# nutdb/nutdb

Hardware: AMD Instinct MI355X
Metric: rows/sec filter->group-by on 1e9-row i64/f64; achieved HBM GB/s vs peak (higher is better)
Workload: dtype i64+f64; 1 GPU; tpch_q1_shape_filter_groupby; columns=6 x 8 B (i64/f64), groups=6, bytes_per_row=48, rows_per_gpu=1000000000, parallelism=single GPU, gpu=AMD Radeon Graphics, kernel_launches=387

## Files before the change

nutdb_amd/csrc/agg_kernel.hpp:

```cpp
#pragma once

#include "agg_ops.hpp"

namespace nut {

enum { CTL_CLAIMED = 0, CTL_SPECIAL = 1, CTL_LOCK = 2, CTL_NDENSE = 3 };
constexpr uint32_t kNoDense = 0xFFFFFFFFu;
constexpr uint32_t kDirect = 256;

struct LTable {
  uint64_t *slot, *agg;
  i64x2 *k12;
  uint32_t *did, *dslot, *ctl;
  uint32_t *dmap;
  uint64_t *priv;
  uint32_t *spill;
  uint32_t *shist;
};

__host__ __device__ inline size_t lds_layout(uint32_t cap, int nk, int na, bool privm, int P, int bd,
                                             size_t *o_k12, size_t *o_did, size_t *o_dslot, size_t *o_ctl,
                                             size_t *o_priv) {
  const size_t stride = cap + 1;
  size_t o = stride * 8 * (1 + (size_t)na);
// ... 434 lines not shown
          }
        }
      });
    }
  }
  if (p.sp_counts) {
    spill_rows<NK, S>(p, lt, kk1, kk2, sl, av, vm);
    return;
  }
#pragma unroll
  for (int r = 0; r < R; ++r) {
    if (sl[r] == -1 && NK == 1 && p.dense) {
      atomicOr(&p.gt->ctl[1], 4u);
    } else if (sl[r] == -1) {
      uint64_t g[8] = {0, 0, 0, 0, 0, 0, 0, 0};
      uint32_t m = 0;
#pragma unroll
      for (int a = 0; a < S::MA && a < 8; ++a) g[a] = av[a][r], m |= vm[a][r] ? 1u << a : 0u;
      g_row<NK>(p.gt, (int64_t)kk1[r], (int64_t)kk2[r], m, g[0], g[1], g[2], g[3], g[4], g[5], g[6], g[7]);
    }
  }
}

template <int NK, bool PRIV, int BD, class S, int VEC>
__global__ __launch_bounds__(BD) void agg_kernel(AggArgs p) {
  extern __shared__ __attribute__((aligned(16))) uint64_t smem[];
  const uint32_t cap = p.lds_cap;
  const uint32_t stride = cap + 1;
  const int na = S::na(p);
  LTable lt;
  {
    size_t o_k12, o_did, o_dslot, o_ctl, o_priv;
    lds_layout(cap, NK, na, PRIV, p.priv, BD, &o_k12, &o_did, &o_dslot, &o_ctl, &o_priv);
    char *b = (char *)smem;
    lt.slot = (uint64_t *)b;
    lt.agg = lt.slot + stride;
    lt.k12 = (i64x2 *)(b + o_k12);
    lt.did = PRIV ? (uint32_t *)(b + o_did) : nullptr;
    lt.dslot = (uint32_t *)(b + o_dslot);
    lt.dmap = PRIV ? lt.dslot + kPrivMax : nullptr;
    lt.ctl = (uint32_t *)(b + o_ctl);
    lt.priv = (uint64_t *)(b + o_priv);
  }
  __shared__ uint32_t s_spill;
  __shared__ uint32_t s_shist[256];
  lt.spill = &s_spill;
// ... 163 lines not shown
        continue;
      }
      if (base == ~0ull) continue;
      const uint64_t pos = base + r;
      t.slot[pos] = wd;
#pragma unroll
      for (int a = 0; a < S::MA; ++a)
        if (a < na) t.agg[a * gstr + pos] = lt.agg[a * stride + s];
    }
    return;
  }
  for (uint32_t s = threadIdx.x; s < stride; s += BD) {
    const uint64_t wd = lt.slot[s];
    const bool occ = s < cap ? wd != kEmpty : lt.ctl[CTL_SPECIAL] != 0u;
    if (!occ) continue;
    const int64_t k1 = NK == 1 ? (int64_t)(s < cap ? wd : kEmpty) : lt.k12[s].x;
    const int64_t k2 = NK == 1 ? 0 : lt.k12[s].y;
    const int64_t gs = g_find<NK>(t, key_hash<NK>(k1, k2), k1, k2);
    if (gs < 0) continue;
#pragma unroll
    for (int a = 0; a < S::MA; ++a)
      if (a < na) agg_merge_word(&t.agg[a * gstr + gs], S::kind(p, a), lt.agg[a * stride + s]);
  }
}

}
```

nutdb_amd/csrc/agg_ops.hpp:

```cpp
#pragma once

#include "gtable.hpp"

namespace nut {

constexpr int kPrivMax = 8;
constexpr int kMaxCols = NUT_MAX_PROG_COLS;
constexpr int kMaxConst = 64;

struct AggArgs {
  uint64_t n;
  const uint64_t *keys[2];
  const uint64_t *pred_col[NUT_MAX_PRED];
  uint64_t pred_k[NUT_MAX_PRED];
  int32_t pred_type[NUT_MAX_PRED];
  int32_t pred_op[NUT_MAX_PRED];
  const uint64_t *val_col[kMaxCols];
  int32_t npred, nvals, naggs;
  uint32_t kinds;
  int32_t expr[NUT_MAX_AGGS];
  int32_t arg[NUT_MAX_AGGS][3];
  uint32_t lds_cap;
  uint32_t lds_limit;
  int32_t lds_log2;
  int32_t priv;
  int32_t vec;
  int32_t nokey;
  int32_t pred_nset[NUT_MAX_PRED];
  uint64_t pred_set[NUT_MAX_PRED][NUT_MAX_SET];
  uint64_t kc[kMaxConst];
  const GTable *gt;
  uint64_t *sp_cols[3 + NUT_MAX_VALS];
  unsigned long long *sp_counts;
  unsigned long long *sp_hist;
  uint64_t sp_region;
  int32_t sp_map[NUT_MAX_AGGS];
  const uint64_t *seg_off;
  const uint64_t *seg_end;
  const uint64_t *seg_cut;
  int32_t dense, pad_;
  unsigned long long *dcount;
  uint64_t dregion, dbase;
};

struct NoProg {
  static constexpr bool kProg = false;
  template <class V>
  __device__ static bool where(const AggArgs &, const V &, int, bool &) { return true; }
  template <class V>
  __device__ static uint64_t value(const AggArgs &, int, const V &, int, bool &) { return 0; }
  template <class V>
  __device__ static bool valid(const AggArgs &, int, const V &, int, bool &) { return true; }
};

template <class S>
__host__ __device__ constexpr int col_type(int c) {
  if constexpr (S::kProg) return (int)((S::kColTypes >> (4 * c)) & 15u);
  else return NUT_T_I64;
}
template <class S>
__host__ __device__ constexpr bool shape_narrow() {
  for (int c = 0; c < S::MV; ++c)
    if (type_width(col_type<S>(c)) < 8) return true;
  return false;
}
// ... 184 lines not shown
```

nutdb_amd/csrc/aggregate.hip:

```cpp
#include <stdlib.h>
#include <string.h>

#include <algorithm>
#include <chrono>
#include <mutex>
#include <thread>
#include <vector>

#include "agg_kernel.hpp"
#include "gpart.hpp"
#include "fold.hpp"
#include "heavy.hpp"
#include "sort.hpp"
#include "jit.hpp"
#include "select_kernel.hpp"

using namespace nut;

struct nut_groups {
  nut_ctx *ctx = nullptr;
  int nk = 1, naggs = 0;
  int32_t kinds[NUT_MAX_AGGS] = {0};
  GTable gt{};
  GTable *dev_gt = nullptr;
  void *mem = nullptr;
  size_t mem_bytes = 0;
  unsigned long long *dev_cursors = nullptr;
  uint64_t *dev_segbase = nullptr;
  bool dense = false;
  uint32_t ctl_cache[4] = {0, 0, 0, 0};
  bool ctl_valid = false;
};

namespace {

int ilog2(uint64_t v) {
  int r = 0;
  while ((1ull << r) < v) ++r;
  return r;
}

uint32_t pack_kinds(const int32_t *k, int n) {
  uint32_t p = 0;
  for (int a = 0; a < n; ++a) p |= (uint32_t)(k[a] & 15) << (4 * a);
  return p;
}

nut_status validate(const nut_agg_spec *s) {
  if (!s) return fail(NUT_ERR_INVALID_ARG, "nut_groupby: spec is NULL");
  if (s->nkeys < 0 || s->nkeys > 2) return fail(NUT_ERR_UNSUPPORTED, "nut_groupby: 0, 1 or 2 key columns supported");
  if (s->npred < 0 || s->npred > NUT_MAX_PRED) return fail(NUT_ERR_UNSUPPORTED, "nut_groupby: too many predicate terms");
  if (s->nvals < 0 || s->nvals > NUT_MAX_VALS) return fail(NUT_ERR_UNSUPPORTED, "nut_groupby: too many value columns");
  if (s->naggs < 0 || s->naggs > NUT_MAX_AGGS) return fail(NUT_ERR_UNSUPPORTED, "nut_groupby: too many aggregates");
  for (int k = 0; k < NUT_MAX_KEYS; ++k) {
// ... 69 lines not shown
        return fail(NUT_ERR_UNSUPPORTED, "nut_groupby: arithmetic expressions need f64 columns");
    }
  }
  return NUT_OK;
}

int32_t kind_of(const nut_agg_spec *s, int a) {
  int op = s->agg_op[a];
  if (op == NUT_AGG_COUNT) return AK_COUNT;
  bool i64 = s->agg_expr[a] == NUT_EX_COL && s->val_type[s->agg_arg[a][0]] == NUT_T_I64;
  if (s->prog_mode) {
    int32_t t = NUT_PT_F64;
    (void)prog_check(&s->agg_val[a], s->prog_col_type, s->nprog_cols, &t);
    i64 = t != NUT_PT_F64;
  }
  switch (op) {
    case NUT_AGG_SUM: return i64 ? AK_SUM_I64 : AK_SUM_F64;
    case NUT_AGG_MIN: return i64 ? AK_MIN_I64 : AK_MIN_F64;
    default: return i64 ? AK_MAX_I64 : AK_MAX_F64;
  }
}

nut_status alloc_table(nut_groups *g, uint64_t cap) {
  g->ctl_valid = false;
  const uint64_t stride = cap + 1;
  const uint64_t arena = g->nk == 2 ? cap + 65536 : 0;
  size_t off = 0;
  auto carve = [&](size_t bytes) {
    size_t o = off;
    off += (bytes + 255) & ~size_t(255);
    return o;
  };
  size_t o_slot = carve(stride * 8);
  size_t o_agg = carve(stride * 8 * (size_t)std::max(g->naggs, 1));
  size_t o_a1 = carve(arena * 8 + 8);
  size_t o_a2 = carve(arena * 8 + 8);
  size_t o_ctl = carve(64);
  const int nsh_log2 = cap >= (1ull << 18) ? 8 : 0;
  const uint32_t nsh = 1u << nsh_log2;
  size_t o_sh = carve((size_t)nsh * 2 * 16 * 4);
  size_t o_gt = carve(sizeof(GTable));
  size_t o_cur = carve(64 * 8);
  size_t o_seg = carve(128 * 8);
  if (!(g->mem && g->mem_bytes >= off)) {
    if (g->mem) (void)hipFree(g->mem);
    g->mem = nullptr;
    nut_status ps = pool_take(g->ctx, off, &g->mem, &g->mem_bytes);
    if (ps) return ps;
  }
  char *b = (char *)g->mem;
  GTable &t = g->gt;
  t.slot = (uint64_t *)(b + o_slot);
  t.agg = (uint64_t *)(b + o_agg);
  t.ak1 = (int64_t *)(b + o_a1);
  t.ak2 = (int64_t *)(b + o_a2);
  t.ctl = (uint32_t *)(b + o_ctl);
  t.shard = (uint32_t *)(b + o_sh);
  t.nsh_log2 = nsh_log2;
  t.cap = cap;
  t.log2cap = ilog2(cap);
  t.limit = (uint32_t)std::min<uint64_t>(cap - cap / 4, 0xFFFFFFF0ull);
  t.arena_cap = (uint32_t)std::min<uint64_t>(arena, 0xFFFFFFF0ull);
  t.limit_sh = nsh == 1 ? t.limit : t.limit / nsh + t.limit / nsh / 16;
  t.arena_sh = t.arena_cap / nsh;
  t.naggs = g->naggs;
  t.kinds = pack_kinds(g->kinds, g->naggs);
  g->dev_gt = (GTable *)(b + o_gt);
  g->dev_cursors = (unsigned long long *)(b + o_cur);
  g->dev_segbase = (uint64_t *)(b + o_seg);
  hipStream_t st = g->ctx->stream;
  NUT_HIP(hipMemsetAsync(t.ctl, 0, 64, st));
  NUT_HIP(hipMemsetAsync(t.shard, 0, (size_t)nsh * 2 * 16 * 4, st));
  NUT_HIP(hipMemcpyAsync(g->dev_gt, &g->gt, sizeof(GTable), hipMemcpyHostToDevice, st));
  uint64_t blocks = std::min<uint64_t>((stride + 255) / 256, (uint64_t)g->ctx->num_cus * 8);
  hipLaunchKernelGGL(gtable_init_kernel, dim3((unsigned)blocks), dim3(256), 0, st, (const GTable *)g->dev_gt, g->nk);
  NUT_HIP(hipGetLastError());
  return NUT_OK;
}

nut_status read_ctl(nut_groups *g, uint32_t *ctl4) {
  if (g->ctl_valid) {
    memcpy(ctl4, g->ctl_cache, 16);
    return NUT_OK;
  }
  nut_ctx *c = g->ctx;
  hipLaunchKernelGGL(gtable_sum_kernel, dim3(1), dim3(256), 0, c->stream, (const GTable *)g->dev_gt);
  NUT_HIP(hipGetLastError());
  NUT_HIP(hipMemcpyAsync(c->host_pinned, g->gt.ctl, 16, hipMemcpyDeviceToHost, c->stream));
  NUT_HIP(hipStreamSynchronize(c->stream));
  memcpy(ctl4, c->host_pinned, 16);
  memcpy(g->ctl_cache, ctl4, 16);
  g->ctl_valid = true;
  return NUT_OK;
}

using KernelFn = void (*)(AggArgs);
enum { SHAPE_GENERIC = 0, SHAPE_Q1, SHAPE_SUM, SHAPE_SUMCOUNT, SHAPE_ALL4 };

template <class S>
bool shape_matches(const nut_agg_spec *s, const int32_t *kinds, const AggArgs &a) {
  if (s->npred != S::MP || s->nvals != S::MV || s->naggs != S::MA) return false;
  for (int i = 0; i < S::MA; ++i) {
    if (kinds[i] != (int)((S::kKinds >> (4 * i)) & 15u)) return false;
    if (a.expr[i] != (int)((S::kExprs >> (4 * i)) & 15u)) return false;
    const int nargs = a.expr[i] == NUT_EX_COL ? 1 : a.expr[i] == NUT_EX_MUL_1M_1P ? 3 : 2;
    for (int j = 0; j < 3; ++j) {
      int want = (int)((S::kArgs >> (6 * i + 2 * j)) & 3u);
// ... 63 lines not shown
constexpr int kPrivShapes[3][2] = {{192, 2}, {128, 3}, {128, 4}};
struct PrivShape {
  int shape = -1;
  double ms[3] = {-1, -1, -1};
  double cost_ms = 0;
};
static PrivShape g_priv_shape[64];
static std::mutex g_priv_mu;
static PrivShape priv_shape_of(int dev) {
  std::lock_guard<std::mutex> lk(g_priv_mu);
  return dev >= 0 && dev < 64 ? g_priv_shape[dev] : PrivShape{};
}

constexpr size_t kAggLdsMax = 160 * 1024 - 2048;
uint32_t agg_lcap(nut_ctx *c, int nk, int na, uint64_t group_hint, bool seg) {
  const uint64_t want = group_hint ? (uint64_t)c->opt[seg ? NUT_OPT_GB_SEG_SLOTS : NUT_OPT_AGG_SLOTS] * group_hint : 4096;
  uint32_t lcap = 32;
  while (lcap < want && lds_bytes(lcap * 2, nk, na, false, 0, kBdShared) <= kAggLdsMax) lcap *= 2;
  return group_hint > 8ull * lcap ? 0 : lcap;
}

nut_status launch_agg(nut_groups *g, const nut_agg_spec *s, uint64_t group_hint, const int32_t *kinds,
                      LaunchExtra *ex = nullptr) {
  g->ctl_valid = false;
  nut_ctx *c = g->ctx;
  if (s->n == 0) return NUT_OK;
  AggArgs a;
  memset(&a, 0, sizeof(a));
  a.n = s->n;
  a.nokey = s->nkeys == 0 ? 1 : 0;
  a.keys[0] = (const uint64_t *)(s->nkeys && !s->key_prog[0].n ? s->keys[0] : nullptr);
  a.keys[1] = s->nkeys == 2 && !s->key_prog[1].n ? (const uint64_t *)s->keys[1] : a.keys[0];
  a.npred = s->npred;
  for (int t = 0; t < s->npred; ++t) {
    a.pred_col[t] = (const uint64_t *)s->pred_col[t];
    a.pred_type[t] = s->pred_type[t];
    a.pred_op[t] = s->pred_op[t];
    if (s->pred_type[t] == NUT_T_I64) a.pred_k[t] = (uint64_t)s->pred_i64[t];
    else memcpy(&a.pred_k[t], &s->pred_f64[t], 8);
    if (s->pred_op[t] >= NUT_IN) {
      a.pred_nset[t] = s->pred_nset[t];
      for (int i = 0; i < s->pred_nset[t]; ++i) a.pred_set[t][i] = (uint64_t)s->pred_set[t][i];
    }
  }
  a.nvals = s->nvals;
  for (int v = 0; v < s->nvals; ++v) a.val_col[v] = (const uint64_t *)s->val_col[v];
  if (s->prog_mode) {
// ... 34 lines not shown
  if (lcap && group_hint && group_hint <= (uint64_t)kPrivMax && na > 0 && !(ex && ex->seg_off)) {
    P = (int)group_hint;
    if (lds_bytes(lcap, g->nk, na, true, P, kBdPriv) > lds_max / 2) P = 0;
  }
  const bool priv = P > 0;
  const int shape = detect_shape(s, kinds, a);
  const bool q1_tuned = priv && ((shape == SHAPE_Q1 && !s->prog_mode && a.vec) || s->prog_mode);
  const bool q1_fused = q1_tuned && !s->prog_mode;
  int pbd = 192, pblocks = 2;
  if (q1_fused) {
    const int k = c->priv_probe >= 0 ? c->priv_probe : priv_shape_of(c->device).shape;
    if (k >= 0) pbd = kPrivShapes[k][0], pblocks = kPrivShapes[k][1];
  }
  if (ex && ex->dry) {
    ex->q1_fused = q1_fused;
    return NUT_OK;
  }
  const int bd = !priv ? kBdShared : !q1_tuned ? kBdPriv : c->opt[NUT_OPT_PRIV_BD] ? (int)c->opt[NUT_OPT_PRIV_BD] : pbd;
  a.lds_cap = lcap;
  a.lds_limit = lcap - lcap / 4;
  a.lds_log2 = lcap ? ilog2(lcap) : 0;
  a.priv = P;
  a.gt = g->dev_gt;
  const size_t lb = lds_bytes(lcap, g->nk, na, priv, P, bd);
  int blocks_per_cu = lb ? (int)std::max<size_t>(1, std::min<size_t>(bd == 512 ? 4 : 8, lds_max / lb)) : 4;
  if (q1_tuned)
    blocks_per_cu = std::min<int>(blocks_per_cu, c->opt[NUT_OPT_PRIV_BLOCKS] ? (int)c->opt[NUT_OPT_PRIV_BLOCKS]
                                                 : q1_fused ? pblocks : 2);
  if (!priv && c->opt[NUT_OPT_AGG_BLOCKS]) blocks_per_cu = std::min<int>(blocks_per_cu, (int)c->opt[NUT_OPT_AGG_BLOCKS]);
  uint64_t pairs = (s->n + 1) / 2;
  uint64_t blocks = std::min<uint64_t>((uint64_t)c->num_cus * blocks_per_cu, (pairs + bd - 1) / bd);
  if (blocks == 0) blocks = 1;
  if (ex && ex->seg_off) {
    a.seg_off = ex->seg_off;
    a.seg_end = ex->seg_end;
    a.seg_cut = ex->seg_cut;
    a.dense = ex->dense && g->nk == 1 ? 1 : 0;
    blocks = ex->nseg;
    if (ex->dcount) {
      if (!a.dense || !lcap || ex->dregion < (uint64_t)lcap + 1)
        return fail(NUT_ERR_INVALID_ARG, "launch_agg: dense staging region smaller than the block table");
      a.dcount = ex->dcount;
      a.dregion = ex->dregion;
      a.dbase = ex->dbase;
    }
  }
  if (ex && ex->spill) {
    a.sp_region = 2ull * bd * ((pairs + blocks * bd - 1) / (blocks * bd));
    ex->blocks = blocks;
    ex->region = a.sp_region;
  }
  if (s->prog_mode) {
    JitShape js;
    nut_status st = jit_shape(s, kinds, js);
    if (st) return st;
    if (js.consts.size() > (size_t)kMaxConst)
      return fail(NUT_ERR_UNSUPPORTED, "nut_groupby: more than 64 distinct expression constants");
    for (size_t i = 0; i < js.consts.size(); ++i) a.kc[i] = js.consts[i];
    hipFunction_t fn;
    st = jit_kernel(jit_unit(js.src, g->nk, priv, bd, sizeof(AggArgs)), true, &fn);
    if (st) return st;
    size_t asz = sizeof(a);
    void *cfg[] = {HIP_LAUNCH_PARAM_BUFFER_POINTER, &a, HIP_LAUNCH_PARAM_BUFFER_SIZE, &asz, HIP_LAUNCH_PARAM_END};
    c->timer.begin(c->stream, NUT_KERNEL_AGGREGATE);
    hipError_t e = hipModuleLaunchKernel(fn, (unsigned)blocks, 1, 1, (unsigned)bd, 1, 1, (unsigned)lb, c->stream,
                                         nullptr, cfg);
    c->timer.end(c->stream);
    if (e != hipSuccess) return hip_fail(e, "hipModuleLaunchKernel (expression kernel)");
    return NUT_OK;
  }
  KernelFn fn = pick_kernel(g->nk, priv, shape, a.vec != 0, bd);
  NUT_HIP(hipFuncSetAttribute((const void *)fn, hipFuncAttributeMaxDynamicSharedMemorySize, (int)lds_max));
  c->timer.begin(c->stream, NUT_KERNEL_AGGREGATE);
  hipLaunchKernelGGL(fn, dim3((unsigned)blocks), dim3(bd), lb, c->stream, a);
  c->timer.end(c->stream);
  NUT_HIP(hipGetLastError());
  return NUT_OK;
}

uint64_t table_cap_for(uint64_t groups) {
  uint64_t cap = 1024;
  while (cap < 2 * groups) cap *= 2;
  return cap;
}

nut_status ensure_room(nut_groups *g, uint64_t extra) {
  uint32_t ctl[4];
  nut_status st = read_ctl(g, ctl);
  if (st) return st;
  uint64_t need = (uint64_t)ctl[0] + extra + 1;
  const uint64_t slack = g->gt.nsh_log2 ? need / 8 : 0;
  if (!g->dense && need + slack <= g->gt.limit && (g->nk == 1 || (uint64_t)ctl[3] + extra + slack <= g->gt.arena_cap))
    return NUT_OK;
  nut_groups fresh;
  fresh.ctx = g->ctx;
  fresh.nk = g->nk;
  fresh.naggs = g->naggs;
  memcpy(fresh.kinds, g->kinds, sizeof(g->kinds));
  st = alloc_table(&fresh, table_cap_for(need));
  if (st) return st;
  nut_ctx *c = g->ctx;
  uint64_t stride = g->gt.cap + 1;
  uint64_t blocks = std::min<uint64_t>((stride + 255) / 256, (uint64_t)c->num_cus * 8);
  hipLaunchKernelGGL(rehash_kernel, dim3((unsigned)blocks), dim3(256), 0, c->stream, (const GTable *)g->dev_gt,
                     (const GTable *)fresh.dev_gt, g->nk);
  NUT_HIP(hipGetLastError());
  NUT_HIP(hipStreamSynchronize(c->stream));
  (void)hipFree(g->mem);
  g->mem = fresh.mem;
  g->mem_bytes = fresh.mem_bytes;
  g->gt = fresh.gt;
  g->dev_gt = fresh.dev_gt;
  g->ctl_valid = false;
  g->dev_cursors = fresh.dev_cursors;
  g->dev_segbase = fresh.dev_segbase;
  g->dense = false;
  fresh.mem = nullptr;
  return NUT_OK;
}

constexpr uint64_t kGpMinGroups = 1ull << 16;

struct GpMeta {
  nut_ctx *c;
  size_t off = 0;
  std::vector<std::vector<char>> keep;
  static size_t al(size_t x) { return (x + 255) & ~size_t(255); }
  nut_status begin(size_t total) {
    off = 0;
    total += 16 * 256;
    if (total > c->gp_meta.bytes) {
      NUT_HIP(hipStreamSynchronize(c->stream));
      nut_status s = c->gp_meta.reserve(total);
      if (s) return s;
    }
    return NUT_OK;
// ... 325 lines not shown
  c->timer.end(st);
  nut_agg_spec s2;
  memset(&s2, 0, sizeof(s2));
  s2.n = n;
  s2.nkeys = nk;
  s2.keys[0] = (const int64_t *)fin[1];
  s2.keys[1] = nk == 2 ? (const int64_t *)fin[2] : nullptr;
  s2.nvals = nv;
  s2.naggs = na;
  for (int j = 0; j < NUT_MAX_VALS; ++j)
    if (vmap[j] >= 0) {
      s2.val_col[vmap[j]] = fin[3 + vmap[j]];
      s2.val_type[vmap[j]] = s->val_type[j];
    }
  for (int a = 0; a < na; ++a) {
    s2.agg_op[a] = s->agg_op[a];
    s2.agg_expr[a] = NUT_EX_COL;
    if (s->agg_op[a] != NUT_AGG_COUNT) s2.agg_arg[a][0] = vmap[s->agg_arg[a][0]];
  }
  return gp_aggregate(g, mm, parts, s2, g->kinds, group_hint);
}

nut_status alloc_stage(nut_groups *g, uint64_t slots) {
  g->ctl_valid = false;
  size_t off = 0;
  auto carve = [&](size_t bytes) {
    size_t o = off;
    off += (bytes + 255) & ~size_t(255);
    return o;
  };
  const size_t o_slot = carve(slots * 8), o_agg = carve(slots * 8 * (size_t)std::max(g->naggs, 1));
  const size_t o_ctl = carve(64), o_sh = carve(16 * 4), o_gt = carve(sizeof(GTable)), o_cur = carve(64 * 8),
               o_seg = carve(128 * 8);
  if (!(g->mem && g->mem_bytes >= off)) {
    if (g->mem) (void)hipFree(g->mem);
    g->mem = nullptr;
    nut_status ps = pool_take(g->ctx, off, &g->mem, &g->mem_bytes);
    if (ps) return ps;
  }
  char *b = (char *)g->mem;
  GTable &t = g->gt;
  memset(&t, 0, sizeof(t));
  t.slot = (uint64_t *)(b + o_slot);
  t.agg = (uint64_t *)(b + o_agg);
  t.ctl = (uint32_t *)(b + o_ctl);
  t.shard = (uint32_t *)(b + o_sh);
  t.cap = slots - 1;
// ... 795 lines not shown
  g->naggs = s->naggs;
  for (int a = 0; a < s->naggs; ++a) g->kinds[a] = kind_of(s, a);
  if (s->nkeys == 0) group_hint = 1;
  uint64_t cap = table_cap_for(group_hint ? group_hint : 8192);
  const int64_t gp = c->opt[NUT_OPT_GB_PARTITION];
  c->gb_path = NUT_GB_ONCHIP;
  c->gb_levels = c->gb_optimistic = 0;
  if (s->nkeys >= 1 && s->n && gp != 0 && (gp == 1 || (group_hint >= kGpMinGroups && s->n >= 4 * group_hint))) {
    bool used = false;
    st = alloc_table(g, cap);
    if (!st) st = groupby_partitioned(g, s, group_hint, &used);
    if (st) {
      nut_groups_free(g);
      return st;
    }
    if (used) {
      *out = g;
      return NUT_OK;
    }
  }
  for (int attempt = 0;; ++attempt) {
    st = alloc_table(g, cap);
    if (!st && attempt == 0) st = probe_priv_shape(g, s, group_hint, cap);
    if (!st) st = launch_agg(g, s, group_hint, g->kinds);
    uint32_t ctl[4] = {0, 0, 0, 0};
    if (!st) st = read_ctl(g, ctl);
    if (st) {
      nut_groups_free(g);
      return st;
    }
    if (ctl[1] & 2u) {
      nut_groups_free(g);
      return fail(NUT_ERR_INVALID_ARG, "nut_groupby: division by zero in an expression");
    }
    if (!(ctl[1] & 1u)) break;
    if (cap >= (1ull << 34) || attempt > 12) {
      nut_groups_free(g);
      return fail(NUT_ERR_OOM, "nut_groupby: group table would exceed device memory");
    }
    cap *= 4;
    group_hint = std::max<uint64_t>(group_hint, ctl[0]);
  }
  *out = g;
  return NUT_OK;
}

nut_status nut_groupby_accumulate(nut_ctx *c, const nut_agg_spec *s, nut_groups *g) {
// ... 406 lines not shown
  }
  for (int a = 0; a < g->naggs; ++a) {
    const int k = g->kinds[a];
    const bool f64 = k == AK_SUM_F64 || k == AK_MIN_F64 || k == AK_MAX_F64;
    const void *col = seg + (uint64_t)(g->nk + a) * c;
    s->agg_op[a] = (k == AK_MIN_F64 || k == AK_MIN_I64) ? NUT_AGG_MIN
                   : (k == AK_MAX_F64 || k == AK_MAX_I64) ? NUT_AGG_MAX : NUT_AGG_SUM;
    if (prog) {
      s->prog_col[a] = col;
      s->prog_col_type[a] = f64 ? NUT_T_F64 : NUT_T_I64;
      nodes[a] = nut_prog_node{NUT_P_COL, a, 0};
      s->agg_val[a] = nut_prog{1, &nodes[a]};
    } else {
      s->val_col[a] = col;
      s->val_type[a] = f64 ? NUT_T_F64 : NUT_T_I64;
      s->agg_expr[a] = NUT_EX_COL;
      s->agg_arg[a][0] = a;
    }
  }
}

}

extern "C" {

nut_status nut_groups_to_host(nut_groups *g, int64_t *keys, uint64_t *aggs, uint64_t cap) {
  if (!g) return fail(NUT_ERR_INVALID_ARG, "nut_groups_to_host: NULL argument");
  uint64_t n;
  nut_status st = nut_groups_size(g, &n);
  if (st) return st;
  if (n > cap)
    return fail(NUT_ERR_CAPACITY, "nut_groups_to_host: capacity " + std::to_string(cap) + " < " +
                                      std::to_string(n) + " groups");
  if (n == 0) return NUT_OK;
  if (!keys || (g->naggs && !aggs)) return fail(NUT_ERR_INVALID_ARG, "nut_groups_to_host: NULL output");
  nut_ctx *c = g->ctx;
  DeviceGuard dg(c->device);
  const int w = g->nk + g->naggs;
  uint64_t *dev = nullptr;
  NUT_HIP(hipMallocAsync((void **)&dev, (size_t)w * n * 8, c->stream));
  st = nut_groups_to_device(g, dev, n);
  if (st) {
    (void)hipFreeAsync(dev, c->stream);
    return st;
  }
  if (g->nk == 1 && n >= (1u << 16)) {
    const uint64_t saved_bytes = c->sort_bytes;
    const uint32_t saved_levels = c->sort_levels;
    uint64_t *buf = nullptr;
    const size_t nb = (size_t)n * 8;
    NUT_HIP(hipMallocAsync((void **)&buf, nb * (2 + (size_t)g->naggs), c->stream));
    int64_t *sorted = (int64_t *)buf, *dk = (int64_t *)(buf + n);
    uint64_t *da = buf + 2 * n;
    st = msd_sort_i64(c, (const int64_t *)dev, sorted, n, 0x8000000000000000ull);
    c->sort_bytes = saved_bytes;
    c->sort_levels = saved_levels;
    uint64_t *bstart = nullptr;
    if (!st) {
// ... 30 lines not shown
  std::sort(order.begin(), order.end(), [&](uint64_t x, uint64_t y) {
    int64_t a0 = (int64_t)h[x], b0 = (int64_t)h[y];
    if (a0 != b0) return a0 < b0;
    if (nk == 2) return (int64_t)h[n + x] < (int64_t)h[n + y];
    return false;
  });
  for (uint64_t i = 0; i < n; ++i) {
    uint64_t src = order[i];
    for (int j = 0; j < nk; ++j) keys[i * nk + j] = (int64_t)h[(size_t)j * n + src];
    for (int a = 0; a < g->naggs; ++a) aggs[i * g->naggs + a] = h[(size_t)(nk + a) * n + src];
  }
  return NUT_OK;
}

constexpr uint64_t kSmallTail = 1ull << 16;
nut_status groupby_small_to_host(nut_ctx *c, const nut_agg_spec *s, uint64_t group_hint, int64_t *keys,
                                 uint64_t *aggs, uint64_t cap, uint64_t *n_out, bool *done) {
  *done = false;
  const int64_t gp = c->opt[NUT_OPT_GB_PARTITION];
  if (s->nkeys == 0 || !s->n) return NUT_OK;
  if (gp == 1 || (gp != 0 && group_hint >= kGpMinGroups && s->n >= 4 * group_hint)) return NUT_OK;
  const uint64_t tcap = table_cap_for(group_hint ? group_hint : 8192);
  if (tcap + 1 > kSmallTail) return NUT_OK;
  nut_groups *g = new nut_groups();
  struct Free {
    nut_groups *g;
    ~Free() { nut_groups_free(g); }
  } free_g{g};
  g->ctx = c;
  g->nk = s->nkeys;
  g->naggs = s->naggs;
  for (int a = 0; a < s->naggs; ++a) g->kinds[a] = kind_of(s, a);
  c->gb_path = NUT_GB_ONCHIP;
  c->gb_levels = c->gb_optimistic = 0;
  nut_status st = alloc_table(g, tcap);
  if (!st) st = probe_priv_shape(g, s, group_hint, tcap);
  if (!st) st = launch_agg(g, s, group_hint, g->kinds);
  if (st) return st;
  const int nk = g->nk, na = g->naggs, w = nk + na;
  const uint64_t stride = g->gt.cap + 1;
  for (auto &b : c->stage)
    if (!b) NUT_HIP(hipHostMalloc((void **)&b, kStageBytes, hipHostMallocDefault));
  if ((stride * w + 2) * 8 > kStageBytes) return NUT_OK;
  uint64_t *dev = nullptr;
  NUT_HIP(hipMallocAsync((void **)&dev, (size_t)stride * w * 8, c->stream));
  struct FreeDev {
    uint64_t *p;
    hipStream_t s;
    ~FreeDev() { (void)hipFreeAsync(p, s); }
  } free_dev{dev, c->stream};
  uint64_t *host = (uint64_t *)c->stage[0];
  hipLaunchKernelGGL(gtable_sum_kernel, dim3(1), dim3(256), 0, c->stream, (const GTable *)g->dev_gt);
  NUT_HIP(hipMemcpyAsync(host, g->gt.ctl, 16, hipMemcpyDeviceToHost, c->stream));
  NUT_HIP(hipMemsetAsync(g->dev_cursors, 0, 64 * 8, c->stream));
  const uint64_t blocks = std::min<uint64_t>((stride + GT_CHUNK - 1) / GT_CHUNK, (uint64_t)c->num_cus * 8);
  hipLaunchKernelGGL(gtable_compact_kernel, dim3((unsigned)blocks), dim3(256), 0, c->stream, (const GTable *)g->dev_gt,
                     nk, dev, stride, g->dev_cursors, 1, (const uint64_t *)nullptr);
  NUT_HIP(hipGetLastError());
  NUT_HIP(hipMemcpyAsync(host + 2, dev, (size_t)stride * w * 8, hipMemcpyDeviceToHost, c->stream));
  NUT_HIP(hipStreamSynchronize(c->stream));
  uint32_t ctl[4];
  memcpy(ctl, host, 16);
  if (ctl[1] & 2u) return fail(NUT_ERR_INVALID_ARG, "nut_groupby: division by zero in an expression");
  if (ctl[1] & 1u) return NUT_OK;
  const uint64_t n = (uint64_t)ctl[0] + (nk == 1 && ctl[2] ? 1 : 0);
  *done = true;
  *n_out = n;
  if (n > cap)
    return fail(NUT_ERR_CAPACITY, "nut_groupby_to_host: capacity " + std::to_string(cap) + " < " + std::to_string(n) +
                                      " groups");
  const uint64_t *h = host + 2;
  std::vector<uint32_t> order(n);
  for (uint64_t i = 0; i < n; ++i) order[i] = (uint32_t)i;
  std::sort(order.begin(), order.end(), [&](uint32_t x, uint32_t y) {
    const int64_t a0 = (int64_t)h[x], b0 = (int64_t)h[y];
    if (a0 != b0) return a0 < b0;
    return nk == 2 && (int64_t)h[stride + x] < (int64_t)h[stride + y];
  });
  for (uint64_t i = 0; i < n; ++i) {
    const uint64_t src = order[i];
    for (int j = 0; j < nk; ++j) keys[i * nk + j] = (int64_t)h[(size_t)j * stride + src];
    for (int a = 0; a < na; ++a) aggs[i * na + a] = h[(size_t)(nk + a) * stride + src];
  }
  return NUT_OK;
}

nut_status nut_groupby_to_host(nut_ctx *c, const nut_agg_spec *s, uint64_t group_hint, int64_t *keys, uint64_t *aggs,
                               uint64_t cap, uint64_t *n_out) {
  if (!c || !n_out) return fail(NUT_ERR_INVALID_ARG, "nut_groupby_to_host: NULL argument");
  *n_out = 0;
  nut_status st = validate(s);
  if (st) return st;
  DeviceGuard dg(c->device);
  st = groupby_ordered(c, s, group_hint, keys, aggs, cap, n_out);
  if (st != NUT_ERR_UNSUPPORTED) return st;
  *n_out = 0;
  bool done = false;
  if (keys && (aggs || !s->naggs)) {
    st = groupby_small_to_host(c, s, group_hint, keys, aggs, cap, n_out, &done);
    if (st || done) return st;
  }
  nut_groups *g = nullptr;
  st = nut_groupby(c, s, group_hint, &g);
  if (st) return st;
  uint64_t n = 0;
  st = nut_groups_size(g, &n);
// ... 71 lines not shown
```

nutdb_amd/csrc/api.hip:

```cpp
#include <stdio.h>
#include <string.h>

#include <algorithm>
#include <thread>

#include "common.hpp"

namespace nut {

static thread_local std::string g_last_error;

void set_error(const std::string &msg) { g_last_error = msg; }

nut_status fail(nut_status st, const std::string &msg) {
  g_last_error = msg;
  return st;
}

nut_status hip_fail(hipError_t e, const char *what) {
  g_last_error = std::string(what) + ": " + hipGetErrorName(e) + " (" + hipGetErrorString(e) + ")";
  return e == hipErrorOutOfMemory ? NUT_ERR_OOM : NUT_ERR_HIP;
}

nut_status Scratch::reserve(size_t need, bool grow) {
// ... 237 lines not shown
}

}

extern "C" {

void nut_ctx_destroy(nut_ctx *c) {
  if (!c) return;
  DeviceGuard g(c->device);
  (void)hipStreamSynchronize(c->stream);
  c->filter_state.release();
  c->sort_tmp.release();
  c->sort_tmp2.release();
  c->sort_status.release();
  c->sort_meta.release();
  c->gp_data.release();
  c->gp_meta.release();
  c->misc.release();
  c->timer.release();
  for (auto &b : c->stage)
    if (b) (void)hipHostFree(b);
  if (c->tbl_pool) (void)hipFree(c->tbl_pool);
  if (c->host_pinned) (void)hipHostFree(c->host_pinned);
  if (c->own_stream) (void)hipStreamDestroy(c->own_stream);
  if (c->copy_stream) (void)hipStreamDestroy(c->copy_stream);
  if (c->aux_stream) (void)hipStreamDestroy(c->aux_stream);
  if (c->order_stream) (void)hipStreamDestroy(c->order_stream);
  delete c;
}

nut_status nut_ctx_set_stream(nut_ctx *c, void *s) {
  if (!c) return fail(NUT_ERR_INVALID_ARG, "nut_ctx_set_stream: ctx is NULL");
  c->stream = (hipStream_t)s;
  return NUT_OK;
}

nut_status nut_ctx_sync(nut_ctx *c) {
  if (!c) return fail(NUT_ERR_INVALID_ARG, "nut_ctx_sync: ctx is NULL");
  DeviceGuard g(c->device);
  NUT_HIP(hipStreamSynchronize(c->stream));
  return NUT_OK;
}

nut_status nut_ctx_memcpy(nut_ctx *c, void *dst, const void *src, size_t bytes) {
  if (!c || (bytes && (!dst || !src))) return fail(NUT_ERR_INVALID_ARG, "nut_ctx_memcpy: NULL argument");
  if (bytes == 0) return NUT_OK;
// ... 130 lines not shown
```

nutdb_amd/csrc/common.hpp:

```cpp
#pragma once

#ifndef __HIPCC_RTC__
#include <hip/hip_runtime.h>
#include <stdint.h>

#include <string>
#include <vector>
#endif

#include "nutexec.h"

namespace nut {

constexpr int kWave = 64;
constexpr uint64_t kGolden = 0x9E3779B97F4A7C15ull;
constexpr uint64_t kPoolSalt = 0x5DEECE66D2545F49ull;
constexpr uint64_t kEmpty = 0x8000000000000000ull;

__host__ __device__ __forceinline__ uint64_t mix64(uint64_t z) {
  z = (z ^ (z >> 30)) * 0xBF58476D1CE4E5B9ull;
  z = (z ^ (z >> 27)) * 0x94D049BB133111EBull;
  return z ^ (z >> 31);
}
__host__ __device__ __forceinline__ uint64_t gen_u64(uint64_t seed, uint64_t row) {
// ... 191 lines not shown
  nut::Scratch sort_tmp2;
  nut::Scratch sort_status;
  void *sort_status_seen = nullptr;
  size_t sort_status_clean = 0;
  uint32_t sort_epoch = 0;
  uint64_t sort_bytes = 0;
  uint32_t sort_levels = 0;
  nut::Scratch sort_meta;
  nut::Scratch gp_data;
  nut::Scratch gp_meta;
  nut::Scratch misc;
  uint64_t *host_pinned = nullptr;
  char *stage[2] = {nullptr, nullptr};
  void *tbl_pool = nullptr;
  size_t tbl_pool_bytes = 0;
  nut::KernelTimer timer;
  int64_t opt[NUT_OPT_COUNT] = {-1, 0, 1, 1, 8, 1, 0, 0, 2, 1, 6, 1, 0, 0, 0, 0, 0, 0, 0, 1, 1, 1, 1, 1024, 4, 32};
  int priv_probe = -1;
  uint32_t gb_path = 0, gb_levels = 0, gb_optimistic = 0;
  uint64_t gb_overflow_rows = 0;
  uint32_t gb_heavy_keys = 0;
  uint64_t gb_heavy_rows = 0;
  uint32_t gb_decline = 0;
};

namespace nut {
struct DeviceGuard {
  int prev = -1;
  explicit DeviceGuard(int dev) {
    (void)hipGetLastError();
    if (hipGetDevice(&prev) != hipSuccess) prev = -1;
    if (prev != dev) (void)hipSetDevice(dev);
  }
  ~DeviceGuard() {
    int cur;
    if (prev >= 0 && hipGetDevice(&cur) == hipSuccess && cur != prev) (void)hipSetDevice(prev);
    (void)hipGetLastError();
  }
};
}
#else
}
#endif
```

nutdb_amd/csrc/gtable.hpp:

```cpp
#pragma once

#include "common.hpp"

namespace nut {

enum AggKind : int32_t {
  AK_SUM_F64 = 0,
  AK_SUM_I64 = 1,
  AK_COUNT = 2,
  AK_MIN_F64 = 3,
  AK_MAX_F64 = 4,
  AK_MIN_I64 = 5,
  AK_MAX_I64 = 6,
};

constexpr uint64_t kEmpty2 = ~0ull;

__host__ __device__ inline uint64_t agg_init(int kind) {
  switch (kind) {
    case AK_MIN_F64: return ~0ull;
    case AK_MAX_F64: return 0ull;
    case AK_MIN_I64: return 0x7FFFFFFFFFFFFFFFull;
    case AK_MAX_I64: return 0x8000000000000000ull;
    default: return 0ull;
// ... 84 lines not shown
        }
        cur = __hip_atomic_compare_exchange_strong(&t.slot[s], &cur, word, __ATOMIC_RELEASE,
                                                   __ATOMIC_RELAXED, __HIP_MEMORY_SCOPE_AGENT)
                  ? kEmpty2
                  : cur;
        if (cur == kEmpty2) {
          if (atomicAdd(&t.shard[(s & ((1u << t.nsh_log2) - 1)) * 16], 1u) >= t.limit_sh) atomicOr(&t.ctl[1], 1u);
          return (int64_t)s;
        }
      }
      if ((uint32_t)(cur >> 32) == tag) {
        uint32_t j = (uint32_t)cur;
        if ((int64_t)rmw_load((uint64_t *)&t.ak1[j]) == k1 && (int64_t)rmw_load((uint64_t *)&t.ak2[j]) == k2)
          return (int64_t)s;
      }
    }
    s = (s + 1) & (t.cap - 1);
  }
  atomicOr(&t.ctl[1], 1u);
  return -1;
}


__global__ void gtable_init_kernel(const GTable *__restrict__ gtp, int nk) {
  const GTable t = *gtp;
  const uint64_t stride = t.cap + 1;
  const uint64_t empty = nk == 1 ? kEmpty : kEmpty2;
  for (uint64_t s = (uint64_t)blockIdx.x * blockDim.x + threadIdx.x; s < stride;
       s += (uint64_t)gridDim.x * blockDim.x) {
    t.slot[s] = empty;
    for (int a = 0; a < t.naggs; ++a) t.agg[a * stride + s] = agg_init(kind_at(t.kinds, a));
  }
}

__device__ __forceinline__ bool slot_keys(const GTable &t, int nk, uint64_t s, uint64_t &k1, uint64_t &k2) {
  if (nk == 1) {
    if (s == t.cap) {
      k1 = kEmpty;
      k2 = 0;
      return t.ctl[2] != 0u;
    }
    k1 = t.slot[s];
    k2 = 0;
    return k1 != kEmpty;
  }
  if (s == t.cap) return false;
  uint64_t w = t.slot[s];
  if (w == kEmpty2) return false;
  k1 = (uint64_t)t.ak1[(uint32_t)w];
  k2 = (uint64_t)t.ak2[(uint32_t)w];
  return true;
}
// ... 142 lines not shown
```

Baseline: 130.9 billion rows/s.

## Finalize small group-by results in last aggregation block into mapped host memory

The last block to finish the aggregation kernel, chosen with a device ticket counter, now compacts the global hash table and writes counts, keys and aggregates into a pinned, device-mapped host buffer. The host then skips the separate sum kernel, device allocation and copy. Table initialisation also folds the ctl/shard memsets and the GTable upload into the init kernel, and hipFuncSetAttribute is called once per device and kernel. This cuts launches and synchronisations per query, in exchange for a serial finish tail in one block and writes across PCIe from the kernel.

```diff
diff --git a/nutdb_amd/csrc/agg_kernel.hpp b/nutdb_amd/csrc/agg_kernel.hpp
--- a/nutdb_amd/csrc/agg_kernel.hpp
+++ b/nutdb_amd/csrc/agg_kernel.hpp
@@ -480,6 +480,78 @@
   }
 }
 
+constexpr int kFinHeader = 4;
+constexpr uint64_t kFinMaxCap = 4096;
+constexpr int kFinPer = 8;
+
+template <int NK>
+__device__ __noinline__ void finish_result(const GTable *__restrict__ gtp, uint64_t *__restrict__ fin,
+                                           uint32_t *s_fin) {
+  const GTable t = *gtp;
+  const uint64_t gstr = t.cap + 1;
+  const uint32_t tid = threadIdx.x, bd = blockDim.x;
+  if (tid == 0) {
+    const uint32_t nsh = 1u << t.nsh_log2;
+    uint32_t c = 0, a = 0;
+    for (uint32_t i = 0; i < nsh; ++i) {
+      c += rmw_load(&t.shard[i * 16]);
+      a += rmw_load(&t.shard[(nsh + i) * 16]);
+    }
+    t.ctl[0] = c;
+    t.ctl[3] = a;
+    s_fin[0] = c;
+    s_fin[1] = rmw_load(&t.ctl[1]);
+    s_fin[2] = rmw_load(&t.ctl[2]);
+    s_fin[3] = a;
+    s_fin[4] = 0;
+  }
+  __syncthreads();
+  const bool special = s_fin[2] != 0u;
+  if (!(s_fin[1] & 1u)) {
+    uint64_t *out = fin + kFinHeader;
+    for (uint64_t c0 = 0; c0 < gstr; c0 += (uint64_t)bd * kFinPer) {
+      uint64_t wd[kFinPer];
+#pragma unroll
+      for (int i = 0; i < kFinPer; ++i) {
+        const uint64_t sl = c0 + (uint64_t)i * bd + tid;
+        wd[i] = sl < t.cap ? rmw_load(&t.slot[sl]) : (NK == 1 ? kEmpty : kEmpty2);
+      }
+#pragma unroll
+      for (int i = 0; i < kFinPer; ++i) {
+        const uint64_t sl = c0 + (uint64_t)i * bd + tid;
+        const bool occ = NK == 1 ? (sl < t.cap ? wd[i] != kEmpty : (sl == t.cap && special))
+                                 : (sl < t.cap && wd[i] != kEmpty2);
+        const uint64_t m = __ballot(occ);
+        if (!m) continue;
+        const int leader = __builtin_ctzll(m);
+        uint32_t b = 0;
+        if ((tid & 63u) == (uint32_t)leader) b = atomicAdd(&s_fin[4], (uint32_t)__popcll(m));
+        const uint64_t pos = __shfl(b, leader, 64) + lane_rank(m);
+        if (!occ) continue;
+        if (NK == 1) {
+          out[pos] = wd[i];
+        } else {
+          out[pos] = rmw_load((uint64_t *)&t.ak1[(uint32_t)wd[i]]);
+          out[gstr + pos] = rmw_load((uint64_t *)&t.ak2[(uint32_t)wd[i]]);
+        }
+        for (int a = 0; a < t.naggs; ++a) {
+          uint64_t x = rmw_load(&t.agg[a * gstr + sl]);
+          const int kind = kind_at(t.kinds, a);
+          if (kind == AK_MIN_F64 || kind == AK_MAX_F64) x = ord_to_f64(x);
+          out[(uint64_t)(NK + a) * gstr + pos] = x;
+        }
+      }
+    }
+  }
+  __syncthreads();
+  if (tid == 0) {
+    fin[0] = (uint64_t)s_fin[0] | (uint64_t)s_fin[1] << 32;
+    fin[1] = (uint64_t)s_fin[2] | (uint64_t)s_fin[3] << 32;
+    fin[2] = s_fin[4];
+    fin[3] = 0;
+  }
+}
+
 template <int NK, bool PRIV, int BD, class S, int VEC>
 __global__ __launch_bounds__(BD) void agg_kernel(AggArgs p) {
   extern __shared__ __attribute__((aligned(16))) uint64_t smem[];
@@ -689,6 +761,23 @@
     for (int a = 0; a < S::MA; ++a)
       if (a < na) agg_merge_word(&t.agg[a * gstr + gs], S::kind(p, a), lt.agg[a * stride + s]);
   }
-}
-
-}
+  if (p.fin) {
+    uint32_t *s_fin = s_shist;
+    asm volatile("s_waitcnt vmcnt(0)" ::: "memory");
+    __syncthreads();
+    if (threadIdx.x == 0) {
+      const bool last = __hip_atomic_fetch_add(&t.ctl[kCtlTicket], 1u, __ATOMIC_RELAXED, __HIP_MEMORY_SCOPE_AGENT) ==
+                        gridDim.x - 1;
+      if (last) {
+        atomicExch(&t.ctl[kCtlTicket], 0u);
+        __builtin_amdgcn_fence(__ATOMIC_ACQUIRE, "agent");
+        asm volatile("s_waitcnt vmcnt(0)" ::: "memory");
+      }
+      s_fin[5] = last ? 1u : 0u;
+    }
+    __syncthreads();
+    if (s_fin[5]) finish_result<NK>(p.gt, p.fin, s_fin);
+  }
+}
+
+}
diff --git a/nutdb_amd/csrc/agg_ops.hpp b/nutdb_amd/csrc/agg_ops.hpp
--- a/nutdb_amd/csrc/agg_ops.hpp
+++ b/nutdb_amd/csrc/agg_ops.hpp
@@ -41,6 +41,7 @@
   int32_t dense, pad_;
   unsigned long long *dcount;
   uint64_t dregion, dbase;
+  uint64_t *fin;
 };
 
 struct NoProg {
diff --git a/nutdb_amd/csrc/aggregate.hip b/nutdb_amd/csrc/aggregate.hip
--- a/nutdb_amd/csrc/aggregate.hip
+++ b/nutdb_amd/csrc/aggregate.hip
@@ -4,7 +4,9 @@
 #include <algorithm>
 #include <chrono>
 #include <mutex>
+#include <set>
 #include <thread>
+#include <utility>
 #include <vector>
 
 #include "agg_kernel.hpp"
@@ -30,6 +32,12 @@
   bool dense = false;
   uint32_t ctl_cache[4] = {0, 0, 0, 0};
   bool ctl_valid = false;
+  std::vector<uint64_t> rows;
+  uint64_t rows_n = 0;
+  bool rows_valid = false;
+  bool want_fin = false;
+  bool fin_pending = false;
+  void touch() { ctl_valid = rows_valid = false; }
 };
 
 namespace {
@@ -145,7 +153,7 @@
 }
 
 nut_status alloc_table(nut_groups *g, uint64_t cap) {
-  g->ctl_valid = false;
+  g->touch();
   const uint64_t stride = cap + 1;
   const uint64_t arena = g->nk == 2 ? cap + 65536 : 0;
   size_t off = 0;
@@ -192,12 +200,48 @@
   g->dev_cursors = (unsigned long long *)(b + o_cur);
   g->dev_segbase = (uint64_t *)(b + o_seg);
   hipStream_t st = g->ctx->stream;
-  NUT_HIP(hipMemsetAsync(t.ctl, 0, 64, st));
-  NUT_HIP(hipMemsetAsync(t.shard, 0, (size_t)nsh * 2 * 16 * 4, st));
-  NUT_HIP(hipMemcpyAsync(g->dev_gt, &g->gt, sizeof(GTable), hipMemcpyHostToDevice, st));
   uint64_t blocks = std::min<uint64_t>((stride + 255) / 256, (uint64_t)g->ctx->num_cus * 8);
-  hipLaunchKernelGGL(gtable_init_kernel, dim3((unsigned)blocks), dim3(256), 0, st, (const GTable *)g->dev_gt, g->nk);
+  hipLaunchKernelGGL(gtable_init_kernel, dim3((unsigned)blocks), dim3(256), 0, st, g->gt, g->dev_gt, g->nk);
   NUT_HIP(hipGetLastError());
+  return NUT_OK;
+}
+
+constexpr size_t kFinWords = kFinHeader + (size_t)(kFinMaxCap + 1) * (NUT_MAX_KEYS + NUT_MAX_AGGS);
+nut_status fin_buffer(nut_ctx *c) {
+  if (c->fin_host) return NUT_OK;
+  uint64_t *h = nullptr, *d = nullptr;
+  NUT_HIP(hipHostMalloc((void **)&h, kFinWords * 8, hipHostMallocDefault));
+  const hipError_t e = hipHostGetDevicePointer((void **)&d, h, 0);
+  if (e != hipSuccess) {
+    (void)hipHostFree(h);
+    return hip_fail(e, "hipHostGetDevicePointer (result buffer)");
+  }
+  c->fin_host = h;
+  c->fin_dev = d;
+  return NUT_OK;
+}
+
+nut_status take_fin(nut_groups *g, uint32_t *ctl4) {
+  nut_ctx *c = g->ctx;
+  g->fin_pending = false;
+  NUT_HIP(hipStreamSynchronize(c->stream));
+  const uint64_t *h = c->fin_host;
+  ctl4[0] = (uint32_t)h[0];
+  ctl4[1] = (uint32_t)(h[0] >> 32);
+  ctl4[2] = (uint32_t)h[1];
+  ctl4[3] = (uint32_t)(h[1] >> 32);
+  memcpy(g->ctl_cache, ctl4, 16);
+  g->ctl_valid = true;
+  if (ctl4[1]) return NUT_OK;
+  const uint64_t n = h[2], stride = g->gt.cap + 1;
+  if (n > stride || n != (uint64_t)ctl4[0] + (g->nk == 1 && ctl4[2] ? 1 : 0))
+    return fail(NUT_ERR_HIP, "nut_groupby: the kernel's result header is inconsistent");
+  const int w = g->nk + g->naggs;
+  g->rows.resize((size_t)w * n);
+  for (int col = 0; col < w && n; ++col)
+    memcpy(&g->rows[(size_t)col * n], h + kFinHeader + (size_t)col * stride, n * 8);
+  g->rows_n = n;
+  g->rows_valid = true;
   return NUT_OK;
 }
 
@@ -206,6 +250,7 @@
     memcpy(ctl4, g->ctl_cache, 16);
     return NUT_OK;
   }
+  if (g->fin_pending) return take_fin(g, ctl4);
   nut_ctx *c = g->ctx;
   hipLaunchKernelGGL(gtable_sum_kernel, dim3(1), dim3(256), 0, c->stream, (const GTable *)g->dev_gt);
   NUT_HIP(hipGetLastError());
@@ -315,7 +360,8 @@
 
 nut_status launch_agg(nut_groups *g, const nut_agg_spec *s, uint64_t group_hint, const int32_t *kinds,
                       LaunchExtra *ex = nullptr) {
-  g->ctl_valid = false;
+  g->touch();
+  g->fin_pending = false;
   nut_ctx *c = g->ctx;
   if (s->n == 0) return NUT_OK;
   AggArgs a;
@@ -396,6 +442,11 @@
   a.lds_log2 = lcap ? ilog2(lcap) : 0;
   a.priv = P;
   a.gt = g->dev_gt;
+  if (g->want_fin && !ex && lcap && g->gt.cap <= kFinMaxCap) {
+    nut_status fs = fin_buffer(c);
+    if (fs) return fs;
+    a.fin = c->fin_dev;
+  }
   const size_t lb = lds_bytes(lcap, g->nk, na, priv, P, bd);
   int blocks_per_cu = lb ? (int)std::max<size_t>(1, std::min<size_t>(bd == 512 ? 4 : 8, lds_max / lb)) : 4;
   if (q1_tuned)
@@ -441,14 +492,25 @@
                                          nullptr, cfg);
     c->timer.end(c->stream);
     if (e != hipSuccess) return hip_fail(e, "hipModuleLaunchKernel (expression kernel)");
+    g->fin_pending = a.fin != nullptr;
     return NUT_OK;
   }
   KernelFn fn = pick_kernel(g->nk, priv, shape, a.vec != 0, bd);
-  NUT_HIP(hipFuncSetAttribute((const void *)fn, hipFuncAttributeMaxDynamicSharedMemorySize, (int)lds_max));
+  {
+    static std::mutex mu;
+    static std::set<std::pair<int, const void *>> set_up;
+    std::lock_guard<std::mutex> lk(mu);
+    const std::pair<int, const void *> key(c->device, (const void *)fn);
+    if (!set_up.count(key)) {
+      NUT_HIP(hipFuncSetAttribute((const void *)fn, hipFuncAttributeMaxDynamicSharedMemorySize, (int)lds_max));
+      set_up.insert(key);
+    }
+  }
   c->timer.begin(c->stream, NUT_KERNEL_AGGREGATE);
   hipLaunchKernelGGL(fn, dim3((unsigned)blocks), dim3(bd), lb, c->stream, a);
   c->timer.end(c->stream);
   NUT_HIP(hipGetLastError());
+  g->fin_pending = a.fin != nullptr;
   return NUT_OK;
 }
 
@@ -485,7 +547,7 @@
   g->mem_bytes = fresh.mem_bytes;
   g->gt = fresh.gt;
   g->dev_gt = fresh.dev_gt;
-  g->ctl_valid = false;
+  g->touch();
   g->dev_cursors = fresh.dev_cursors;
   g->dev_segbase = fresh.dev_segbase;
   g->dense = false;
@@ -857,7 +919,7 @@
 }
 
 nut_status alloc_stage(nut_groups *g, uint64_t slots) {
-  g->ctl_valid = false;
+  g->touch();
   size_t off = 0;
   auto carve = [&](size_t bytes) {
     size_t o = off;
@@ -1699,7 +1761,9 @@
   for (int attempt = 0;; ++attempt) {
     st = alloc_table(g, cap);
     if (!st && attempt == 0) st = probe_priv_shape(g, s, group_hint, cap);
+    g->want_fin = true;
     if (!st) st = launch_agg(g, s, group_hint, g->kinds);
+    g->want_fin = false;
     uint32_t ctl[4] = {0, 0, 0, 0};
     if (!st) st = read_ctl(g, ctl);
     if (st) {
@@ -2152,6 +2216,22 @@
 
 }
 
+static void rows_to_host(const uint64_t *h, uint64_t n, uint64_t stride, int nk, int na, int64_t *keys,
+                         uint64_t *aggs) {
+  std::vector<uint32_t> order(n);
+  for (uint64_t i = 0; i < n; ++i) order[i] = (uint32_t)i;
+  std::sort(order.begin(), order.end(), [&](uint32_t x, uint32_t y) {
+    const int64_t a0 = (int64_t)h[x], b0 = (int64_t)h[y];
+    if (a0 != b0) return a0 < b0;
+    return nk == 2 && (int64_t)h[stride + x] < (int64_t)h[stride + y];
+  });
+  for (uint64_t i = 0; i < n; ++i) {
+    const uint64_t src = order[i];
+    for (int j = 0; j < nk; ++j) keys[i * nk + j] = (int64_t)h[(size_t)j * stride + src];
+    for (int a = 0; a < na; ++a) aggs[i * na + a] = h[(size_t)(nk + a) * stride + src];
+  }
+}
+
 extern "C" {
 
 nut_status nut_groups_to_host(nut_groups *g, int64_t *keys, uint64_t *aggs, uint64_t cap) {
@@ -2164,6 +2244,10 @@
                                       std::to_string(n) + " groups");
   if (n == 0) return NUT_OK;
   if (!keys || (g->naggs && !aggs)) return fail(NUT_ERR_INVALID_ARG, "nut_groups_to_host: NULL output");
+  if (g->rows_valid) {
+    rows_to_host(g->rows.data(), g->rows_n, g->rows_n, g->nk, g->naggs, keys, aggs);
+    return NUT_OK;
+  }
   nut_ctx *c = g->ctx;
   DeviceGuard dg(c->device);
   const int w = g->nk + g->naggs;
@@ -2240,6 +2324,7 @@
   if (gp == 1 || (gp != 0 && group_hint >= kGpMinGroups && s->n >= 4 * group_hint)) return NUT_OK;
   const uint64_t tcap = table_cap_for(group_hint ? group_hint : 8192);
   if (tcap + 1 > kSmallTail) return NUT_OK;
+  if ((tcap + 1) * (uint64_t)(s->nkeys + s->naggs) * 8 + 16 > kStageBytes) return NUT_OK;
   nut_groups *g = new nut_groups();
   struct Free {
     nut_groups *g;
@@ -2253,13 +2338,29 @@
   c->gb_levels = c->gb_optimistic = 0;
   nut_status st = alloc_table(g, tcap);
   if (!st) st = probe_priv_shape(g, s, group_hint, tcap);
+  g->want_fin = true;
   if (!st) st = launch_agg(g, s, group_hint, g->kinds);
+  g->want_fin = false;
   if (st) return st;
   const int nk = g->nk, na = g->naggs, w = nk + na;
+  if (g->fin_pending) {
+    uint32_t ctl[4];
+    st = take_fin(g, ctl);
+    if (st) return st;
+    if (ctl[1] & 2u) return fail(NUT_ERR_INVALID_ARG, "nut_groupby: division by zero in an expression");
+    if (ctl[1] & 1u) return NUT_OK;
+    const uint64_t n = g->rows_n;
+    *done = true;
+    *n_out = n;
+    if (n > cap)
+      return fail(NUT_ERR_CAPACITY, "nut_groupby_to_host: capacity " + std::to_string(cap) + " < " + std::to_string(n) +
+                                        " groups");
+    rows_to_host(g->rows.data(), n, n, nk, na, keys, aggs);
+    return NUT_OK;
+  }
   const uint64_t stride = g->gt.cap + 1;
   for (auto &b : c->stage)
     if (!b) NUT_HIP(hipHostMalloc((void **)&b, kStageBytes, hipHostMallocDefault));
-  if ((stride * w + 2) * 8 > kStageBytes) return NUT_OK;
   uint64_t *dev = nullptr;
   NUT_HIP(hipMallocAsync((void **)&dev, (size_t)stride * w * 8, c->stream));
   struct FreeDev {
@@ -2287,19 +2388,7 @@
   if (n > cap)
     return fail(NUT_ERR_CAPACITY, "nut_groupby_to_host: capacity " + std::to_string(cap) + " < " + std::to_string(n) +
                                       " groups");
-  const uint64_t *h = host + 2;
-  std::vector<uint32_t> order(n);
-  for (uint64_t i = 0; i < n; ++i) order[i] = (uint32_t)i;
-  std::sort(order.begin(), order.end(), [&](uint32_t x, uint32_t y) {
-    const int64_t a0 = (int64_t)h[x], b0 = (int64_t)h[y];
-    if (a0 != b0) return a0 < b0;
-    return nk == 2 && (int64_t)h[stride + x] < (int64_t)h[stride + y];
-  });
-  for (uint64_t i = 0; i < n; ++i) {
-    const uint64_t src = order[i];
-    for (int j = 0; j < nk; ++j) keys[i * nk + j] = (int64_t)h[(size_t)j * stride + src];
-    for (int a = 0; a < na; ++a) aggs[i * na + a] = h[(size_t)(nk + a) * stride + src];
-  }
+  rows_to_host(host + 2, n, stride, nk, na, keys, aggs);
   return NUT_OK;
 }
 
diff --git a/nutdb_amd/csrc/api.hip b/nutdb_amd/csrc/api.hip
--- a/nutdb_amd/csrc/api.hip
+++ b/nutdb_amd/csrc/api.hip
@@ -283,6 +283,7 @@
     if (b) (void)hipHostFree(b);
   if (c->tbl_pool) (void)hipFree(c->tbl_pool);
   if (c->host_pinned) (void)hipHostFree(c->host_pinned);
+  if (c->fin_host) (void)hipHostFree(c->fin_host);
   if (c->own_stream) (void)hipStreamDestroy(c->own_stream);
   if (c->copy_stream) (void)hipStreamDestroy(c->copy_stream);
   if (c->aux_stream) (void)hipStreamDestroy(c->aux_stream);
diff --git a/nutdb_amd/csrc/common.hpp b/nutdb_amd/csrc/common.hpp
--- a/nutdb_amd/csrc/common.hpp
+++ b/nutdb_amd/csrc/common.hpp
@@ -237,6 +237,7 @@
   uint32_t gb_heavy_keys = 0;
   uint64_t gb_heavy_rows = 0;
   uint32_t gb_decline = 0;
+  uint64_t *fin_host = nullptr, *fin_dev = nullptr;
 };
 
 namespace nut {
diff --git a/nutdb_amd/csrc/gtable.hpp b/nutdb_amd/csrc/gtable.hpp
--- a/nutdb_amd/csrc/gtable.hpp
+++ b/nutdb_amd/csrc/gtable.hpp
@@ -130,12 +130,17 @@
 }
 
 
-__global__ void gtable_init_kernel(const GTable *__restrict__ gtp, int nk) {
-  const GTable t = *gtp;
+constexpr int kCtlWords = 16;
+constexpr int kCtlTicket = 4;
+__global__ void gtable_init_kernel(const GTable t, GTable *__restrict__ dev_gt, int nk) {
   const uint64_t stride = t.cap + 1;
   const uint64_t empty = nk == 1 ? kEmpty : kEmpty2;
-  for (uint64_t s = (uint64_t)blockIdx.x * blockDim.x + threadIdx.x; s < stride;
-       s += (uint64_t)gridDim.x * blockDim.x) {
+  const uint64_t g0 = (uint64_t)blockIdx.x * blockDim.x + threadIdx.x;
+  if (g0 == 0) *dev_gt = t;
+  if (g0 < (uint64_t)kCtlWords) t.ctl[g0] = 0u;
+  const uint64_t nshw = (uint64_t)2 * 16 << t.nsh_log2;
+  for (uint64_t i = g0; i < nshw; i += (uint64_t)gridDim.x * blockDim.x) t.shard[i] = 0u;
+  for (uint64_t s = g0; s < stride; s += (uint64_t)gridDim.x * blockDim.x) {
     t.slot[s] = empty;
     for (int a = 0; a < t.naggs; ++a) t.agg[a * stride + s] = agg_init(kind_at(t.kinds, a));
   }
```

Measured after the change: 131.7 billion rows/s (median of 6 runs). No clear change (+0.7%).
